# nannau/DoWnGAN

Hardware: AMD Instinct MI355X
Metric: train-step samples/sec (G+D+GP) (higher is better)
Workload: dtype bf16

## Files before the change

downgan_amd/csrc/conv_s2dgrad.hip:

```cpp
#include "gg_common.h"

namespace {

constexpr int NT = 512;
constexpr int RING_PIX = 17;
constexpr int RING_PITCH = 288;
constexpr int MASK_OFF = RING_PIX * RING_PITCH;
constexpr int RING_ROW = MASK_OFF + 2 * 32 * 16;
constexpr int RING_CHUNKS = RING_PIX * 16;

struct S2DArgs {
  const char* dy; const char* w; char* dx; const char* mask_bits;
  float slope;
  int Ho, Wo;
  int nstrips, nitems, trips;
};

__device__ __forceinline__ __amdgpu_buffer_rsrc_t uniform_rsrc(const char* p) {
  const unsigned long long b = (unsigned long long)p;
  const unsigned long long u = ((unsigned long long)(unsigned)__builtin_amdgcn_readfirstlane((int)(unsigned)(b >> 32)) << 32) |
                               (unsigned)__builtin_amdgcn_readfirstlane((int)(unsigned)b);
  return __builtin_amdgcn_make_buffer_rsrc((void*)u, 0, (int)DG_OOB_OFF, 0x00020000);
}

// ... 131 lines not shown
          store_pixel<MASK>(acc[0], acc[1], mb[0], a.slope, rY, st_lane + row0 * 256u);
        }
        {
          f32x4_t acc[2] = {f32x4_t{0.f, 0.f, 0.f, 0.f}, f32x4_t{0.f, 0.f, 0.f, 0.f}};
#pragma unroll
          for (int cb = 0; cb < 2; ++cb) {
            const uint4 b01[2] = {frag(sA, 1, cb, 0), frag(sA, 1, cb, 1)};
            tap(cb, 1, b01, acc); tap(cb, 2, b00[cb], acc);
          }
          store_pixel<MASK>(acc[0], acc[1], mb[1], a.slope, rY, st_lane + (row0 + 1) * 256u);
        }
        {
          f32x4_t acc[2] = {f32x4_t{0.f, 0.f, 0.f, 0.f}, f32x4_t{0.f, 0.f, 0.f, 0.f}};
#pragma unroll
          for (int cb = 0; cb < 2; ++cb) {
            const uint4 b10[2] = {frag(sB, 0, cb, 0), frag(sB, 0, cb, 1)};
            tap(cb, 3, b10, acc); tap(cb, 4, b00[cb], acc);
          }
          store_pixel<MASK>(acc[0], acc[1], mb[2], a.slope, rY, st_lane + (row0 + W) * 256u);
        }
      }
      if (filler) *reinterpret_cast<uint4*>(fill_dst + sC) = __builtin_bit_cast(uint4, staged);
      if (mwave) *reinterpret_cast<uint4*>(mfill_dst + sC) = __builtin_bit_cast(uint4, mstaged);
      __syncthreads();
      const int s = sA; sA = sB; sB = sC; sC = s;
    };
    for (int r = 0; r < a.Ho; r += 2) {
      step(r, st0, st1, ms0, ms1);
      if (r + 1 < a.Ho) step(r + 1, st1, st0, ms1, ms0);
    }
  }
}

std::atomic<int> g_s2_stream{1};
std::atomic<int> g_cus{0};

}

template <bool MASK>
__global__ __launch_bounds__(NT, 1) void s2dgrad_stream_kernel(const S2DArgs a) {
  __shared__ __attribute__((aligned(16))) char ring[3 * RING_ROW];
  if (__builtin_amdgcn_readfirstlane(threadIdx.x >> 6) < 4) s2d_run<MASK, true>(a, ring);
  else s2d_run<MASK, false>(a, ring);
}

bool s2dgrad_stream_eligible(const dg_conv_geom* g, const dg_epilogue* ep) {
  if (!g || g->dtype != DG_BF16 || g->stride != 2 || g->pixel_shuffle) return false;
  if (g->N <= 0 || g->H <= 0 || g->W <= 0 || ((g->H | g->W) & 1)) return false;
  if (g->Cin != 128 || g->Cout != 128 || g->ldx != 128 || g->ldy != 128) return false;
  if (!gg_halo_row_step_ok(g->W / 2, g->ldy, g->dtype, 1)) return false;
  if ((long long)g->H * g->W * 256 >= (1ll << 31)) return false;
  if (ep && (ep->bias || ep->has_act || ep->r1 || ep->r2 || ep->mask || ep->accumulate || ep->out_bits || ep->mask_c0 || ep->mask_last ||
             ep->out_q || ep->out_qs || ep->out_u || ep->out_ue || ep->skip_y || ep->out_amax))
    return false;
  return true;
}

int s2dgrad_stream_mode() { return g_s2_stream.load(std::memory_order_relaxed); }

extern "C" int dg_set_s2_dgrad_stream(int on) { return g_s2_stream.exchange(on < 0 ? 0 : on, std::memory_order_relaxed); }

int s2dgrad_stream_launch(const dg_conv_geom* g, const dg_epilogue* ep, const void* dy, const void* w, void* dx, hipStream_t st) {
  if (!dy || !w || !dx) return DG_ERR_BAD_ARG;
  int cus = g_cus.load(std::memory_order_relaxed);
  if (cus <= 0) {
    int dev = 0;
    if (hipGetDevice(&dev) != hipSuccess || hipDeviceGetAttribute(&cus, hipDeviceAttributeMultiprocessorCount, dev) != hipSuccess || cus <= 0)
      return DG_ERR_LAUNCH;
    g_cus.store(cus, std::memory_order_relaxed);
  }
  S2DArgs a{};
  a.dy = (const char*)dy; a.w = (const char*)w; a.dx = (char*)dx;
  a.mask_bits = ep ? (const char*)ep->mask_bits : nullptr;
  a.slope = ep ? ep->mask_slope : 1.f;
  a.Ho = g->H / 2; a.Wo = g->W / 2;
  a.nstrips = (a.Wo + 15) / 16;
  const long long items = (long long)g->N * a.nstrips;
  if (items >= (1ll << 31)) return DG_ERR_BAD_SHAPE;
  a.nitems = (int)items;
  const int mode = s2dgrad_stream_mode();
  int grid = mode > 1 && mode < cus ? mode : cus;
  if (grid > a.nitems) grid = a.nitems;
  a.trips = (a.nitems + grid - 1) / grid;
  g_last_kinds |= 64;
  if (a.mask_bits) hipLaunchKernelGGL(s2dgrad_stream_kernel<true>, dim3(grid), dim3(NT), 0, st, a);
  else hipLaunchKernelGGL(s2dgrad_stream_kernel<false>, dim3(grid), dim3(NT), 0, st, a);
  return dg_check_launch();
}
```

downgan_amd/_lib.py:

```python
from __future__ import annotations

import ctypes as C
import os

_HERE = os.path.dirname(os.path.abspath(__file__))
LIB_PATH = os.environ.get("DG_LIB_OVERRIDE") or os.path.join(_HERE, "csrc", "libdowngan_hip.so")

DG_F32, DG_BF16 = 0, 1
STATUS = {0: "DG_OK", -1: "DG_ERR_BAD_SHAPE", -2: "DG_ERR_BAD_DTYPE", -3: "DG_ERR_BAD_ARG", -4: "DG_ERR_LAUNCH"}


class Epilogue(C.Structure):
    _fields_ = [("bias", C.c_void_p), ("has_act", C.c_int), ("act_slope", C.c_float),
                ("r1", C.c_void_p), ("ldr1", C.c_int64), ("s1", C.c_float),
                ("r2", C.c_void_p), ("ldr2", C.c_int64), ("s2", C.c_float),
                ("mask", C.c_void_p), ("ldmask", C.c_int64), ("mask_slope", C.c_float),
                ("accumulate", C.c_int), ("mask_bits", C.c_void_p), ("out_bits", C.c_void_p),
                ("mask_c0", C.c_int), ("mask_last", C.c_int), ("out_q", C.c_void_p), ("out_qs", C.c_void_p), ("ldqs", C.c_int64),
                ("out_u", C.c_void_p), ("out_ue", C.c_void_p), ("skip_y", C.c_int), ("out_amax", C.c_void_p)]


class ConvGeom(C.Structure):
    _fields_ = [("dtype", C.c_int), ("N", C.c_int), ("H", C.c_int), ("W", C.c_int),
                ("Cin", C.c_int), ("Cout", C.c_int), ("stride", C.c_int), ("cin_real", C.c_int), ("pixel_shuffle", C.c_int),
# ... 103 lines not shown


class DistmapSpec(C.Structure):
    _fields_ = [("speed_u", C.c_int), ("speed_v", C.c_int), ("nthr", C.c_int), ("nring", C.c_int), ("cutoff", C.c_int),
                ("scale", C.c_float * EOF_MAX_C), ("offset", C.c_float * EOF_MAX_C),
                ("thr", (C.c_float * DIST_MAX_THR) * HIST_MAX_OUT)]


class TemporalSpec(C.Structure):
    _fields_ = [("speed_u", C.c_int), ("speed_v", C.c_int), ("nthr", C.c_int), ("ndur", C.c_int), ("nlag", C.c_int),
                ("nbins", C.c_int), ("below", C.c_int * TEMPORAL_MAX_THR), ("lag", C.c_int * TEMPORAL_MAX_LAGS),
                ("scale", C.c_float * EOF_MAX_C), ("offset", C.c_float * EOF_MAX_C),
                ("thr", (C.c_float * TEMPORAL_MAX_THR) * HIST_MAX_OUT), ("lo", (C.c_float * TEMPORAL_MAX_LAGS) * HIST_MAX_OUT),
                ("inv_w", (C.c_float * TEMPORAL_MAX_LAGS) * HIST_MAX_OUT)]


MINMAX_PARTS = 256
_vp, _i, _i64, _f = C.c_void_p, C.c_int, C.c_int64, C.c_float
_PROTOS = {
    "dg_conv3x3_fwd": [C.POINTER(ConvGeom), C.POINTER(Epilogue), _vp, _vp, _vp, _vp],
    "dg_conv3x3_dgrad": [C.POINTER(ConvGeom), C.POINTER(Epilogue), _vp, _vp, _vp, _vp],
    "dg_conv3x3_wgrad": [C.POINTER(ConvGeom), _vp, _vp, _vp, _vp, _vp],
    "dg_conv3x3_wgrad_dense": [_vp, _i, _vp, _vp, _vp, _vp, _vp],
    "dg_conv3x3_wgrad_f8": [C.POINTER(ConvGeom), _vp, _vp, _vp, _vp, _vp, _vp],
    "dg_exp_from_amax": [_vp, _i, _i, _vp, _vp],
    "dg_conv3x3_wgrad_dense_f8": [C.POINTER(ConvGeom), _i, _vp, _vp, _vp, _vp, _vp, _vp],
    "dg_gather_gemm": [C.POINTER(GGDesc), C.POINTER(Epilogue), _vp, _vp, _vp, _vp],
    "dg_conv3x3_plan": [C.POINTER(ConvGeom), _i, C.POINTER(GGDesc)],
    "dg_last_conv_kernels": [],
    "dg_last_wgrad_kernel": [],
    "dg_conv3x3_dgrad_launches": [C.POINTER(ConvGeom)],
    "dg_conv3x3_dgrad_stream_eligible": [C.POINTER(ConvGeom), C.POINTER(Epilogue)],
    "dg_set_s2_dgrad_stream": [C.c_int],
    "dg_colsum": [_i, _vp, _i64, _i64, _i64, _i64, _i, _vp, _vp],
    "dg_colsum_multi": [_i, _vp, _i64, _i64, _i, _i, _vp, _vp],
    "dg_repack_conv_weights": [_i, _i, _vp, _vp, _i, _i, _vp],
    "dg_repack_dense_dgrad": [_i, _vp, _i, _i, _vp, _vp],
    "dg_wgrad_unswap": [_vp, _vp, _i, _i, _vp],
    "dg_linear_fwd": [_i, _vp, _i64, _vp, _i64, _vp, _i, _i, _i, _i64, _vp],
    "dg_linear_dx": [_i, _i, _vp, _i, _vp, _i64, _vp, _i64, _vp, _i64, _f, _i, _i, _i64, _vp],
    "dg_linear_dw": [_i, _vp, _i, _vp, _i64, _vp, _i64, _i, _i, _i64, _vp],
    "dg_linear_dw_wide": [_i, _vp, _i, _vp, _i64, _vp, _i64, _i, _i, _i64, _i, _vp],
    "dg_bias_act": [_i, _vp, _i, _vp, _vp, _i, _i, _i, _i, _f, _vp, _i, _f, _vp],
    "dg_mask_mul": [_i, _vp, _i64, _vp, _i64, _i64, _i, _f, _vp],
    "dg_axpby": [_i, _vp, _i64, _vp, _i64, _f, _vp, _i64, _f, _i64, _i, _vp],
    "dg_gp_interp": [_i, _vp, _vp, _vp, _vp, _i, _i64, _vp],
    "dg_gp_interp_c2": [_i, _vp, _vp, _i64, _vp, _vp, _vp, _vp, _i, _i64, _vp],
    "dg_scale_rows_c2": [_i, _vp, _i64, _vp, _vp, _i, _i64, _vp],
    "dg_sumsq_rows": [_i, _vp, _i, _i64, _vp, _vp],
    "dg_gp_finish": [_vp, _i, _i, _f, _f, _vp, _vp, _vp],
    "dg_scale_rows": [_i, _vp, _vp, _vp, _i, _i64, _vp],
    "dg_l1": [_i, _vp, _i64, _vp, _i64, _i64, _i, _vp, _vp, _i64, _f, _vp, _i64, _vp],
    "dg_sqdiff": [_i, _vp, _i64, _vp, _i64, _i64, _i, _vp, _vp],
    "dg_sum_strided": [_vp, _i, _i, _f, _vp, _vp],
    "dg_fill_col": [_vp, _i, _i, _i, _f, _vp],
    "dg_adam": [_vp, _vp, _vp, _vp, _vp, _i64, _f, _f, _f, _f, _i, _f, _vp],
    "dg_nchw_to_nhwc": [_i, _vp, _vp, _i, _i, _i, _i, _i, _vp],
    "dg_nhwc_to_nchw": [_i, _vp, _i64, _vp, _i, _i, _i, _i, _vp],
    "dg_cast": [_i, _vp, _vp, _i64, _vp],
    "dg_minmax_partial": [_i, _vp, _i64, _i64, _i, _vp, _vp],
    "dg_minmax_finish": [_vp, _i, _vp, _vp],
    "dg_normalise_planar": [_i, _vp, _i, _i, _i, _i64, _i, _vp, _vp, _vp],
    "dg_ssim_level": [_vp, _vp, _i, _i, _i, C.POINTER(SsimParams), _vp, _vp],
    "dg_avgpool2": [_vp, _vp, _i, _i, _i, _vp],
    "dg_msssim_finish": [_vp, _i, _i, C.POINTER(MsssimCombine), _vp, _vp],
    "dg_div_vort_sums": [_i, _vp, _i64, _vp, _i64, _i, _i, _i, _vp, _vp],
# ... 127 lines not shown
```

downgan_amd/csrc/linear.hip:

```cpp
#include "dg_internal.h"
#include <stdlib.h>

template <typename T> struct MmaL;
template <> struct MmaL<bf16_t> {
  static __device__ __forceinline__ void run(const uint4& a, const uint4& b, f32x4_t& c) {
    c = __builtin_amdgcn_mfma_f32_16x16x32_bf16(__builtin_bit_cast(bf16x8_t, a), __builtin_bit_cast(bf16x8_t, b), c, 0, 0, 0);
  }
};
template <> struct MmaL<float> {
  static __device__ __forceinline__ void run(const uint4& a, const uint4& b, f32x4_t& c) {
    c = __builtin_amdgcn_mfma_f32_16x16x4f32(__uint_as_float(a.x), __uint_as_float(b.x), c, 0, 0, 0);
    c = __builtin_amdgcn_mfma_f32_16x16x4f32(__uint_as_float(a.y), __uint_as_float(b.y), c, 0, 0, 0);
    c = __builtin_amdgcn_mfma_f32_16x16x4f32(__uint_as_float(a.z), __uint_as_float(b.z), c, 0, 0, 0);
    c = __builtin_amdgcn_mfma_f32_16x16x4f32(__uint_as_float(a.w), __uint_as_float(b.w), c, 0, 0, 0);
  }
};

typedef __attribute__((ext_vector_type(2))) float dg_f32x2_t;
template <typename T> struct LdX4;
typedef __attribute__((ext_vector_type(2))) unsigned int dg_u32x2_t;
template <> struct LdX4<float> {
  typedef dg_u32x4_t raw;
  static __device__ __forceinline__ raw load(const float* row, unsigned voff) {
    return __builtin_amdgcn_raw_buffer_load_b128(__builtin_amdgcn_make_buffer_rsrc((void*)row, 0, -1, 0x00020000), voff, 0, 0);
// ... 224 lines not shown
        acc[4 * q + e][0] = __builtin_elementwise_fma(d2, wa, acc[4 * q + e][0]);
        acc[4 * q + e][1] = __builtin_elementwise_fma(d2, wb, acc[4 * q + e][1]);
      }
  };
  auto wrow = [&](int o) { return LdX4<T>::load(w + (long long)(o < O ? o : O - 1) * ldw, voff); };
  constexpr int PD = 6;
  typename LdX4<T>::raw wq[PD];
#pragma unroll
  for (int u = 0; u < PD; ++u) wq[u] = wrow(u);
  read_row(d[0], 0);
  for (int o = 0; o < O; o += PD) {
#pragma unroll
    for (int u = 0; u < PD; ++u) {
      read_row(d[(u + 1) & 1], o + u + 1 < O ? o + u + 1 : O);
      landed(d[u & 1]);
      row_fma(wq[u], d[u & 1]);
      wq[u] = wrow(o + u + PD);
    }
  }
#pragma unroll
  for (int b = 0; b < BG; ++b) {
    if (b0 + b >= B) break;
    float v[4] = {acc[b][0][0], acc[b][0][1], acc[b][1][0], acc[b][1][1]};
    if (mask) {
      float mv[4];
      ld4(mask + (long long)(b0 + b) * ldmask + k, mv);
#pragma unroll
      for (int e = 0; e < 4; ++e) v[e] *= leaky_grad(mv[e], slope);
    }
    st4(dx + (long long)(b0 + b) * lddx + k, v);
  }
}

extern "C" int dg_linear_dx(int dtype, int out_dtype, const float* dy, int ldo, const void* w, int64_t ldw, void* dx,
                            int64_t lddx, const void* mask, int64_t ldmask, float mask_slope, int B, int O, int64_t K,
                            void* stream) {
  if (!dy || !w || !dx) return DG_ERR_BAD_ARG;
  if (B <= 0 || O <= 0 || O > 128 || K <= 0 || K % 8 || ldw % 8 || lddx % 8) return DG_ERR_BAD_SHAPE;
  if (mask && ldmask % 8) return DG_ERR_BAD_SHAPE;
  hipStream_t st = reinterpret_cast<hipStream_t>(stream);
  if (K >= 4096 && (long long)K * 4 < (1ll << 32) && B >= 16) {
    dim3 gridw((unsigned)((K / 4 + 255) / 256), (unsigned)((B + 31) / 32));
    if (dtype == DG_F32 && out_dtype == DG_F32) {
      hipLaunchKernelGGL((lin_dx_wide_kernel<float, float>), gridw, dim3(256), 0, st, dy, ldo, (const float*)w, (long long)ldw, (float*)dx,
                         (long long)lddx, (const float*)mask, (long long)ldmask, mask_slope, B, O, (long long)K);
      return dg_check_launch();
    }
    if (dtype == DG_BF16 && out_dtype == DG_BF16) {
      hipLaunchKernelGGL((lin_dx_wide_kernel<bf16_t, bf16_t>), gridw, dim3(256), 0, st, dy, ldo, (const bf16_t*)w, (long long)ldw, (bf16_t*)dx,
                         (long long)lddx, (const bf16_t*)mask, (long long)ldmask, mask_slope, B, O, (long long)K);
      return dg_check_launch();
    }
  }
  constexpr int BG = 16;
  const int epc = dtype == DG_F32 ? 4 : 8;
  dim3 grid((unsigned)((K / epc + 255) / 256), (unsigned)((B + BG - 1) / BG));
  if (dtype == DG_F32 && out_dtype == DG_F32)
    hipLaunchKernelGGL((lin_dx_kernel<float, float, BG>), grid, dim3(256), 0, st, dy, ldo, (const float*)w, ldw,
                       (float*)dx, lddx, (const float*)mask, ldmask, mask_slope, B, O, K);
  else if (dtype == DG_BF16 && out_dtype == DG_BF16)
    hipLaunchKernelGGL((lin_dx_kernel<bf16_t, bf16_t, BG>), grid, dim3(256), 0, st, dy, ldo, (const bf16_t*)w, ldw,
                       (bf16_t*)dx, lddx, (const bf16_t*)mask, ldmask, mask_slope, B, O, K);
  else if (dtype == DG_BF16 && out_dtype == DG_F32)
    hipLaunchKernelGGL((lin_dx_kernel<bf16_t, float, BG>), grid, dim3(256), 0, st, dy, ldo, (const bf16_t*)w, ldw,
                       (float*)dx, lddx, (const bf16_t*)mask, ldmask, mask_slope, B, O, K);
  else
    return DG_ERR_BAD_DTYPE;
  return dg_check_launch();
}

template <typename T, int OT>
__global__ __launch_bounds__(256) void lin_dw_kernel(const float* __restrict__ dy, int ldo, const T* __restrict__ x,
                                                     long long ldx, float* dw, long long lddw, int B, int O,
// ... 84 lines not shown
      for (int j = 0; j < OW; ++j) {
        const float dv = dp[j];
        const dg_f32x2_t d2 = {dv, dv};
        acc[j][0] = __builtin_elementwise_fma(d2, xa, acc[j][0]);
        acc[j][1] = __builtin_elementwise_fma(d2, xb, acc[j][1]);
      }
    };
    const int Bm = B / (2 * UB) * (2 * UB);
    fetch(0, 0);
    for (int b0 = 0; b0 < Bm; b0 += 2 * UB) {
      fetch(1, b0 + UB);
#pragma unroll
      for (int u = 0; u < UB; ++u) row_fma(xr[0][u], b0 + u);
      fetch(0, b0 + 2 * UB);
#pragma unroll
      for (int u = 0; u < UB; ++u) row_fma(xr[1][u], b0 + UB + u);
    }
    for (int b = Bm; b < B; ++b) row_fma(LdX4<T>::load(x + (long long)b * ldx, voff), b);
#pragma unroll
    for (int j = 0; j < OW; ++j) {
      const int o = wave * OW + j;
      if (o >= O) break;
      float4* p = reinterpret_cast<float4*>(dw + (long long)o * lddw + k);
      float4 t = make_float4(acc[j][0][0], acc[j][0][1], acc[j][1][0], acc[j][1][1]);
      if (ACC) {
        const float4 old = *p;
        t.x += old.x; t.y += old.y; t.z += old.z; t.w += old.w;
      }
      *p = t;
    }
  }
}

extern "C" int dg_linear_dw_wide(int dtype, const float* dy, int ldo, const void* x, int64_t ldx, float* dw, int64_t lddw,
                                 int B, int O, int64_t K, int accumulate, void* stream) {
  if (!dy || !x || !dw) return DG_ERR_BAD_ARG;
  if (B <= 0 || B > 128 || O <= 0 || O > 112 || ldo < 112 || K <= 0 || K >= (1ll << 30) || K % 4 || ldx % 4 || lddw % 4 || ldx < K || lddw < K)
    return DG_ERR_BAD_SHAPE;
  if (dtype != DG_F32 && dtype != DG_BF16) return DG_ERR_BAD_DTYPE;
  hipStream_t st = reinterpret_cast<hipStream_t>(stream);
  const long long chunks = (K + 255) / 256;
  const int cpw = chunks >= 8 * 2048 ? 8 : chunks >= 2048 ? 2 : 1;
  const unsigned grid = (unsigned)((chunks + cpw - 1) / cpw);
  constexpr int NWV = 8;
#define DG_LDW(T, ACC)                                                                                                  \
  hipLaunchKernelGGL((lin_dw_wide_kernel<T, ACC, NWV>), dim3(grid), dim3(64 * NWV), 0, st, dy, ldo, (const T*)x, \
                     (long long)ldx, dw, (long long)lddw, B, O, (long long)K, cpw)
  if (dtype == DG_F32) { if (accumulate) DG_LDW(float, true); else DG_LDW(float, false); }
  else { if (accumulate) DG_LDW(bf16_t, true); else DG_LDW(bf16_t, false); }
#undef DG_LDW
  return dg_check_launch();
}
```

include/downgan_hip.h:

```cpp
#ifndef DOWNGAN_HIP_H
#define DOWNGAN_HIP_H

#include <stddef.h>
#include <stdint.h>

#ifdef __cplusplus
extern "C" {
#endif

#define DG_F32 0
#define DG_BF16 1

typedef enum dg_status {
  DG_OK = 0,
  DG_ERR_BAD_SHAPE = -1,
  DG_ERR_BAD_DTYPE = -2,
  DG_ERR_BAD_ARG = -3,
  DG_ERR_LAUNCH = -4
} dg_status;

typedef struct dg_epilogue {
  const float* bias;
  int has_act;
  float act_slope;
// ... 47 lines not shown
                     const void* w_dgrad, void* dx, void* stream);

int dg_conv3x3_wgrad(const dg_conv_geom* g, const void* x, const void* dy, float* dw, float* db,
                     void* stream);

int dg_conv3x3_wgrad_dense(const dg_conv_geom* g, int nconv, const void* x, const void* dy,
                           float* const* dw, float* const* db, void* stream);

int dg_conv3x3_wgrad_f8(const dg_conv_geom* g, const void* xq, const void* ex, const void* dyq, const void* ey, float* dw,
                        void* stream);

int dg_conv3x3_wgrad_dense_f8(const dg_conv_geom* g, int nconv, const void* xq, const void* ex, const void* dyq, const void* ey,
                              float* const* dw, void* stream);

int dg_colsum(int dtype, const void* dy, int64_t rows_outer, int64_t ld_outer, int64_t rows_inner,
              int64_t ld, int C, float* db, void* stream);

int dg_colsum_multi(int dtype, const void* dy, int64_t rows, int64_t ld, int C, int nseg, float* const* db, void* stream);

int dg_gather_gemm(const dg_gg_desc* d, const dg_epilogue* ep, const void* x, const void* w, void* y,
                   void* stream);

int dg_last_conv_kernels(void);

int dg_last_wgrad_kernel(void);

int dg_conv3x3_plan(const dg_conv_geom* g, int kind, dg_gg_desc* out);

int dg_conv3x3_dgrad_launches(const dg_conv_geom* g);

int dg_conv3x3_dgrad_stream_eligible(const dg_conv_geom* g, const dg_epilogue* ep);

int dg_set_s2_dgrad_stream(int on);

int dg_repack_conv_weights(int dtype, int kind, const float* master, void* dst, int CoutP, int CinP,
                           void* stream);
int dg_repack_dense_dgrad(int dtype, const float* const* masters, int nconv, int F, void* dst, void* stream);
int dg_wgrad_unswap(const float* tmp, float* dw, int CoutP, int CinP, void* stream);


int dg_linear_fwd(int dtype, const void* x, int64_t ldx, const void* w, int64_t ldw, float* y,
                  int ldy, int B, int O, int64_t K, void* stream);
int dg_linear_dx(int dtype, int out_dtype, const float* dy, int ldo, const void* w, int64_t ldw,
                 void* dx, int64_t lddx, const void* mask, int64_t ldmask, float mask_slope, int B,
                 int O, int64_t K, void* stream);
int dg_linear_dw(int dtype, const float* dy, int ldo, const void* x, int64_t ldx, float* dw,
                 int64_t lddw, int B, int O, int64_t K, void* stream);
int dg_linear_dw_wide(int dtype, const float* dy, int ldo, const void* x, int64_t ldx, float* dw,
                      int64_t lddw, int B, int O, int64_t K, int accumulate, void* stream);


int dg_bias_act(int out_dtype, const float* in, int ldi, const float* bias, void* out, int ldo,
                int rows, int C, int has_act, float slope, const void* mask, int ldmask,
                float mask_slope, void* stream);
int dg_mask_mul(int dtype, void* u, int64_t ldu, const void* y, int64_t ldy, int64_t rows, int C,
                float slope, void* stream);
int dg_axpby(int dtype, void* out, int64_t ldo, const void* x, int64_t ldx, float a, const void* y,
             int64_t ldy, float b, int64_t rows, int C, void* stream);
int dg_gp_interp(int dtype, const void* real, const void* fake, const float* alpha, void* xhat,
                 int B, int64_t per_img, void* stream);
int dg_gp_interp_c2(int dtype, const void* real, const void* fake, int64_t ld, const float* alpha,
                    void* xhat_c, void* real_c, void* fake_c, int B, int64_t pix_per_img, void* stream);
int dg_scale_rows_c2(int dtype, const void* g, int64_t ld, const float* coef, void* out_c, int B,
                     int64_t pix_per_img, void* stream);
int dg_sumsq_rows(int dtype, const void* g, int B, int64_t per_img, float* ss, void* stream);
int dg_gp_finish(const float* ss, int B, int B_global, float gp_lambda, float weight, float* coef,
// ... 283 lines not shown
```

Baseline: 73.77.

## Add streaming stride-2 dgrad kernel for 256-channel convolutions

Extends the streaming stride-2 transposed-conv data-gradient kernel to Cin=Cout=256, which previously fell back to another path. Each block handles one 64-output-channel slice of a strip and keeps that slice's weights in registers, reloading them only when the slice changes. Row ring buffering in LDS overlaps the next row's load with the MMA work. Work is assigned per XCD so blocks on the same die share strips. The cost is heavy register use for the weight fragments, plus four passes over the input strip, one per channel slice.

After: 73.95 (median of 3 runs). About the same (+0.2%).

```diff
diff --git a/downgan_amd/csrc/conv_s2dgrad.hip b/downgan_amd/csrc/conv_s2dgrad.hip
--- a/downgan_amd/csrc/conv_s2dgrad.hip
+++ b/downgan_amd/csrc/conv_s2dgrad.hip
@@ -187,6 +187,197 @@
   }
 }
 
+constexpr int R2_PITCH = 544;
+constexpr int R2_MASK_OFF = RING_PIX * R2_PITCH;
+constexpr int R2_ROW = R2_MASK_OFF + 2 * 32 * 8;
+
+struct S2D256Args {
+  const char* dy; const char* w; char* dx; const char* mask_bits;
+  float slope;
+  int Ho, Wo;
+  int nstrips, npairs, trips;
+  int per_xcd;
+};
+
+template <bool MASK>
+__device__ __forceinline__ void store_pixel4(const f32x4_t& f, unsigned nib, float slope, __amdgpu_buffer_rsrc_t rY, unsigned off) {
+  float v[4] = {f[0], f[1], f[2], f[3]};
+  if (MASK) {
+#pragma unroll
+    for (int e = 0; e < 4; ++e) v[e] *= ((nib >> e) & 1u) ? 1.f : slope;
+  }
+  EpiIO<bf16_t>::store(v, rY, off);
+}
+
+template <bool MASK, bool C11>
+__device__ __forceinline__ void s2d256_run(const S2D256Args& a, char* ring) {
+  constexpr int NTAP = C11 ? 4 : 5;
+  const int tid = threadIdx.x, lane = tid & 63, q = (tid >> 6) & 3;
+  const int l15 = lane & 15, g = lane >> 4;
+
+  uint4 wr[NTAP * 8];
+  int wslice = -1;
+
+  const int W = 2 * a.Wo;
+  const char* const fb0 = ring + l15 * R2_PITCH + g * 16;
+  const int fill_pix = tid >> 5;
+  char* const fill_dst = ring + fill_pix * R2_PITCH + (tid & 31) * 16;
+  const bool xfiller = C11 && tid < 32;
+  char* const xfill_dst = ring + 16 * R2_PITCH + (tid & 31) * 16;
+
+  for (int trip = 0; trip < a.trips; ++trip) {
+    int pair, s;
+    if (a.per_xcd > 0) {
+      const int j = (int)blockIdx.x >> 3;
+      s = j & 3;
+      pair = (trip * a.per_xcd + (j >> 2)) * 8 + ((int)blockIdx.x & 7);
+    } else {
+      const int item = (int)blockIdx.x + trip * (int)gridDim.x;
+      s = item & 3;
+      pair = item >> 2;
+    }
+    if (pair >= a.npairs) break;
+    if (s != wslice) {
+      wslice = s;
+      constexpr int TW11[4] = {0, 2, 6, 8}, TWX[5] = {4, 3, 5, 1, 7};
+      const int n = 64 * s + 16 * q + l15;
+#pragma unroll
+      for (int cb = 0; cb < 4; ++cb)
+#pragma unroll
+        for (int t = 0; t < NTAP; ++t)
+#pragma unroll
+          for (int kk = 0; kk < 2; ++kk) {
+            const int tw = C11 ? TW11[t] : TWX[t];
+            wr[(cb * NTAP + t) * 2 + kk] =
+                *reinterpret_cast<const uint4*>(a.w + ((long long)n * 2304 + tw * 256 + 64 * cb + 32 * kk + 8 * g) * 2);
+          }
+    }
+    const int img = pair / a.nstrips, x0 = (pair - img * a.nstrips) * 16;
+    const __amdgpu_buffer_rsrc_t rX = uniform_rsrc(a.dy + ((long long)img * a.Ho * a.Wo + x0) * 512);
+    const __amdgpu_buffer_rsrc_t rY = uniform_rsrc(a.dx + ((long long)img * 2 * a.Ho * W + 2 * x0) * 512);
+    const __amdgpu_buffer_rsrc_t rM = uniform_rsrc(MASK ? a.mask_bits + ((long long)img * 2 * a.Ho * W + 2 * x0) * 32 : a.dx);
+    const unsigned fill_off = x0 + fill_pix < a.Wo ? (unsigned)tid * 16u : DG_OOB_OFF;
+    const unsigned xfill_off = (xfiller && x0 + 16 < a.Wo) ? (unsigned)(16 * 512 + tid * 16) : DG_OOB_OFF;
+    const unsigned pix_ok = x0 + l15 < a.Wo ? 0u : DG_OOB_OFF;
+    const unsigned st_lane = pix_ok | (unsigned)(2 * l15 * 512 + 128 * s + 32 * q + 8 * g);
+    auto fetch_row = [&](unsigned off, int rr) {
+      return __builtin_amdgcn_raw_buffer_load_b128(rX, rr < a.Ho ? off + (unsigned)rr * (unsigned)a.Wo * 512u : DG_OOB_OFF, 0, 0);
+    };
+    const bool mwave = MASK && !C11 && __builtin_amdgcn_readfirstlane(tid >> 6) == 5;
+    const int ml = tid & 63;
+    const unsigned mfill_off = 2 * x0 + (ml & 31) < W ? (unsigned)(((ml >> 5) * W + (ml & 31)) * 32 + 8 * s) : DG_OOB_OFF;
+    char* const mfill_dst = ring + R2_MASK_OFF + ml * 8;
+    auto fetch_mask = [&](int k) {
+      return __builtin_amdgcn_raw_buffer_load_b64(rM, k < a.Ho ? mfill_off + (unsigned)(2 * k) * (unsigned)W * 32u : DG_OOB_OFF, 0, 0);
+    };
+    const char* const mrd = ring + R2_MASK_OFF + 2 * l15 * 8 + 2 * q + (g >> 1);
+    const unsigned nsh = 4u * (unsigned)(g & 1);
+    {
+      const u32x4_t r0 = fetch_row(fill_off, 0), r1 = fetch_row(fill_off, 1);
+      *reinterpret_cast<uint4*>(fill_dst) = __builtin_bit_cast(uint4, r0);
+      *reinterpret_cast<uint4*>(fill_dst + R2_ROW) = __builtin_bit_cast(uint4, r1);
+      if constexpr (C11) {
+        const u32x4_t x0r = fetch_row(xfill_off, 0), x1r = fetch_row(xfill_off, 1);
+        if (xfiller) {
+          *reinterpret_cast<uint4*>(xfill_dst) = __builtin_bit_cast(uint4, x0r);
+          *reinterpret_cast<uint4*>(xfill_dst + R2_ROW) = __builtin_bit_cast(uint4, x1r);
+        }
+      }
+      if (mwave) *reinterpret_cast<uint2*>(mfill_dst + R2_ROW) = __builtin_bit_cast(uint2, fetch_mask(0));
+    }
+    u32x4_t st0 = fetch_row(fill_off, 2), st1;
+    u32x4_t xs0 = {0u, 0u, 0u, 0u}, xs1 = {0u, 0u, 0u, 0u};
+    if (xfiller) xs0 = fetch_row(xfill_off, 2);
+    u32x2_t ms0 = {0u, 0u}, ms1 = {0u, 0u};
+    if (mwave) ms0 = fetch_mask(1);
+    __syncthreads();
+    int sA = 0, sB = R2_ROW, sC = 2 * R2_ROW;
+    auto step = [&](int r, const u32x4_t& staged, u32x4_t& nxt, const u32x4_t& xstaged, u32x4_t& xnxt, const u32x2_t& mstaged,
+                    u32x2_t& mnxt) __attribute__((always_inline)) {
+      nxt = fetch_row(fill_off, r + 3);
+      if (xfiller) xnxt = fetch_row(xfill_off, r + 3);
+      if (mwave) mnxt = fetch_mask(r + 2);
+      unsigned mb[3] = {0u, 0u, 0u};
+      if (MASK) {
+        if (C11) {
+          mb[0] = *reinterpret_cast<const unsigned char*>(mrd + sB + 256 + 8);
+        } else {
+          mb[0] = *reinterpret_cast<const unsigned char*>(mrd + sB);
+          mb[1] = *reinterpret_cast<const unsigned char*>(mrd + sB + 8);
+          mb[2] = *reinterpret_cast<const unsigned char*>(mrd + sB + 256);
+        }
+      }
+      const unsigned row0 = (unsigned)(2 * r) * (unsigned)W;
+      __builtin_amdgcn_sched_barrier(0);
+      auto frag = [&](int slot, int sx, int cb, int kk) {
+        return *reinterpret_cast<const uint4*>(fb0 + slot + sx * R2_PITCH + cb * 128 + kk * 64);
+      };
+      if constexpr (C11) {
+        f32x4_t acc = {0.f, 0.f, 0.f, 0.f};
+        uint4 b[2][8];
+        auto read = [&](int cb) {
+#pragma unroll
+          for (int t = 0; t < 4; ++t)
+#pragma unroll
+            for (int kk = 0; kk < 2; ++kk) b[cb & 1][t * 2 + kk] = frag(t < 2 ? sB : sA, (t & 1) ? 0 : 1, cb, kk);
+        };
+        read(0);
+#pragma unroll
+        for (int cb = 0; cb < 4; ++cb) {
+          if (cb < 3) read(cb + 1);
+          __builtin_amdgcn_sched_barrier(0);
+#pragma unroll
+          for (int i = 0; i < 8; ++i) Mma<bf16_t>::run(wr[cb * 8 + i], b[cb & 1][i], acc);
+          __builtin_amdgcn_sched_barrier(0);
+        }
+        store_pixel4<MASK>(acc, mb[0] >> nsh, a.slope, rY, st_lane + (row0 + W + 1) * 512u);
+      } else {
+        f32x4_t a00 = {0.f, 0.f, 0.f, 0.f}, a01 = {0.f, 0.f, 0.f, 0.f}, a10 = {0.f, 0.f, 0.f, 0.f};
+        uint4 b[2][6];
+        auto read = [&](int cb) {
+#pragma unroll
+          for (int kk = 0; kk < 2; ++kk) {
+            b[cb & 1][kk] = frag(sA, 0, cb, kk);
+            b[cb & 1][2 + kk] = frag(sA, 1, cb, kk);
+            b[cb & 1][4 + kk] = frag(sB, 0, cb, kk);
+          }
+        };
+        read(0);
+#pragma unroll
+        for (int cb = 0; cb < 4; ++cb) {
+          if (cb < 3) read(cb + 1);
+          __builtin_amdgcn_sched_barrier(0);
+          const uint4* const bc = b[cb & 1];
+#pragma unroll
+          for (int kk = 0; kk < 2; ++kk) {
+            Mma<bf16_t>::run(wr[cb * 10 + 0 + kk], bc[kk], a00);
+            Mma<bf16_t>::run(wr[cb * 10 + 2 + kk], bc[2 + kk], a01);
+            Mma<bf16_t>::run(wr[cb * 10 + 6 + kk], bc[4 + kk], a10);
+          }
+#pragma unroll
+          for (int kk = 0; kk < 2; ++kk) {
+            Mma<bf16_t>::run(wr[cb * 10 + 4 + kk], bc[kk], a01);
+            Mma<bf16_t>::run(wr[cb * 10 + 8 + kk], bc[kk], a10);
+          }
+          __builtin_amdgcn_sched_barrier(0);
+        }
+        store_pixel4<MASK>(a00, mb[0] >> nsh, a.slope, rY, st_lane + row0 * 512u);
+        store_pixel4<MASK>(a01, mb[1] >> nsh, a.slope, rY, st_lane + (row0 + 1) * 512u);
+        store_pixel4<MASK>(a10, mb[2] >> nsh, a.slope, rY, st_lane + (row0 + W) * 512u);
+      }
+      *reinterpret_cast<uint4*>(fill_dst + sC) = __builtin_bit_cast(uint4, staged);
+      if (xfiller) *reinterpret_cast<uint4*>(xfill_dst + sC) = __builtin_bit_cast(uint4, xstaged);
+      if (mwave) *reinterpret_cast<uint2*>(mfill_dst + sC) = __builtin_bit_cast(uint2, mstaged);
+      __syncthreads();
+      const int sw = sA; sA = sB; sB = sC; sC = sw;
+    };
+    for (int r = 0; r < a.Ho; r += 2) {
+      step(r, st0, st1, xs0, xs1, ms0, ms1);
+      if (r + 1 < a.Ho) step(r + 1, st1, st0, xs1, xs0, ms1, ms0);
+    }
+  }
+}
+
 std::atomic<int> g_s2_stream{1};
 std::atomic<int> g_cus{0};
 
@@ -199,12 +390,19 @@
   else s2d_run<MASK, false>(a, ring);
 }
 
+template <bool MASK>
+__global__ __launch_bounds__(NT, 1) void s2dgrad_stream256_kernel(const S2D256Args a) {
+  __shared__ __attribute__((aligned(16))) char ring[3 * R2_ROW];
+  if (__builtin_amdgcn_readfirstlane(threadIdx.x >> 6) < 4) s2d256_run<MASK, true>(a, ring);
+  else s2d256_run<MASK, false>(a, ring);
+}
+
 bool s2dgrad_stream_eligible(const dg_conv_geom* g, const dg_epilogue* ep) {
   if (!g || g->dtype != DG_BF16 || g->stride != 2 || g->pixel_shuffle) return false;
   if (g->N <= 0 || g->H <= 0 || g->W <= 0 || ((g->H | g->W) & 1)) return false;
-  if (g->Cin != 128 || g->Cout != 128 || g->ldx != 128 || g->ldy != 128) return false;
+  if ((g->Cin != 128 && g->Cin != 256) || g->Cout != g->Cin || g->ldx != g->Cin || g->ldy != g->Cin) return false;
   if (!gg_halo_row_step_ok(g->W / 2, g->ldy, g->dtype, 1)) return false;
-  if ((long long)g->H * g->W * 256 >= (1ll << 31)) return false;
+  if ((long long)g->H * g->W * g->Cin * 2 >= (1ll << 31)) return false;
   if (ep && (ep->bias || ep->has_act || ep->r1 || ep->r2 || ep->mask || ep->accumulate || ep->out_bits || ep->mask_c0 || ep->mask_last ||
              ep->out_q || ep->out_qs || ep->out_u || ep->out_ue || ep->skip_y || ep->out_amax))
     return false;
@@ -223,6 +421,27 @@
     if (hipGetDevice(&dev) != hipSuccess || hipDeviceGetAttribute(&cus, hipDeviceAttributeMultiprocessorCount, dev) != hipSuccess || cus <= 0)
       return DG_ERR_LAUNCH;
     g_cus.store(cus, std::memory_order_relaxed);
+  }
+  const int mode = s2dgrad_stream_mode();
+  if (g->Cin == 256) {
+    S2D256Args a{};
+    a.dy = (const char*)dy; a.w = (const char*)w; a.dx = (char*)dx;
+    a.mask_bits = ep ? (const char*)ep->mask_bits : nullptr;
+    a.slope = ep ? ep->mask_slope : 1.f;
+    a.Ho = g->H / 2; a.Wo = g->W / 2;
+    a.nstrips = (a.Wo + 15) / 16;
+    const long long pairs = (long long)g->N * a.nstrips;
+    if (pairs >= (1ll << 28)) return DG_ERR_BAD_SHAPE;
+    a.npairs = (int)pairs;
+    const int items = 4 * a.npairs;
+    int grid = mode > 1 && mode < cus ? mode : cus;
+    if (grid > items) grid = items;
+    a.per_xcd = grid % 32 == 0 ? grid / 32 : 0;
+    a.trips = a.per_xcd ? (a.npairs + grid / 4 - 1) / (grid / 4) : (items + grid - 1) / grid;
+    g_last_kinds |= 64;
+    if (a.mask_bits) hipLaunchKernelGGL(s2dgrad_stream256_kernel<true>, dim3(grid), dim3(NT), 0, st, a);
+    else hipLaunchKernelGGL(s2dgrad_stream256_kernel<false>, dim3(grid), dim3(NT), 0, st, a);
+    return dg_check_launch();
   }
   S2DArgs a{};
   a.dy = (const char*)dy; a.w = (const char*)w; a.dx = (char*)dx;
@@ -233,7 +452,6 @@
   const long long items = (long long)g->N * a.nstrips;
   if (items >= (1ll << 31)) return DG_ERR_BAD_SHAPE;
   a.nitems = (int)items;
-  const int mode = s2dgrad_stream_mode();
   int grid = mode > 1 && mode < cus ? mode : cus;
   if (grid > a.nitems) grid = a.nitems;
   a.trips = (a.nitems + grid - 1) / grid;
```

## Add MFMA paths for wide linear dx and dw using three-way bf16 splitting

Applied to the files above, without the earlier changes.

Adds MFMA-based kernels for the linear-layer input gradient and the wide weight gradient in bf16. The fp32 dy operand is split into three bf16 terms so the product keeps near-fp32 accuracy, and weight/activation tiles are staged in LDS with a prefetch of the next tile and read with transposed LDS loads. This replaces the scalar FMA row kernels for large K, trading three MFMAs per product and extra LDS traffic for matrix-core throughput. A runtime switch, on by default, allows either path to be disabled.

Result: no change. 73.84 before, 73.98 after, median of 6 (+0.2%).

```diff
diff --git a/downgan_amd/_lib.py b/downgan_amd/_lib.py
--- a/downgan_amd/_lib.py
+++ b/downgan_amd/_lib.py
@@ -159,6 +159,7 @@
     "dg_conv3x3_dgrad_launches": [C.POINTER(ConvGeom)],
     "dg_conv3x3_dgrad_stream_eligible": [C.POINTER(ConvGeom), C.POINTER(Epilogue)],
     "dg_set_s2_dgrad_stream": [C.c_int],
+    "dg_set_linear_mfma": [C.c_int],
     "dg_colsum": [_i, _vp, _i64, _i64, _i64, _i64, _i, _vp, _vp],
     "dg_colsum_multi": [_i, _vp, _i64, _i64, _i, _i, _vp, _vp],
     "dg_repack_conv_weights": [_i, _i, _vp, _vp, _i, _i, _vp],
diff --git a/downgan_amd/csrc/linear.hip b/downgan_amd/csrc/linear.hip
--- a/downgan_amd/csrc/linear.hip
+++ b/downgan_amd/csrc/linear.hip
@@ -280,6 +280,156 @@
   }
 }
 
+constexpr int MX_KT = 256, MX_PITCH = 2 * MX_KT + 16, MX_ROWS = 128;
+constexpr int MX_LDS = MX_ROWS * MX_PITCH;
+#define MX_OOB 0x80000000u
+__device__ __forceinline__ __amdgpu_buffer_rsrc_t mx_rsrc(const void* p) {
+  return __builtin_amdgcn_make_buffer_rsrc((void*)p, 0, (int)MX_OOB, 0x00020000);
+}
+__device__ __forceinline__ bf16x8_t mx_read_tr16(const unsigned char* lo_p, const unsigned char* hi_p) {
+  typedef __attribute__((address_space(3))) s16x4_t* lds_s16x4_ptr;
+  typedef __attribute__((ext_vector_type(8))) short s16x8_t;
+  const s16x4_t lo = __builtin_amdgcn_ds_read_tr16_b64_v4i16((lds_s16x4_ptr)(lo_p));
+  const s16x4_t hi = __builtin_amdgcn_ds_read_tr16_b64_v4i16((lds_s16x4_ptr)(hi_p));
+  const s16x8_t v = {lo[0], lo[1], lo[2], lo[3], hi[0], hi[1], hi[2], hi[3]};
+  return __builtin_bit_cast(bf16x8_t, v);
+}
+__device__ __forceinline__ void mx_split3(const float (&v)[8], bf16x8_t (&t)[3]) {
+  unsigned h[3][8];
+#pragma unroll
+  for (int j = 0; j < 8; ++j) {
+    float r = v[j];
+#pragma unroll
+    for (int s = 0; s < 3; ++s) {
+      h[s][j] = __float_as_uint(r) & 0xffff0000u;
+      r -= __uint_as_float(h[s][j]);
+    }
+  }
+#pragma unroll
+  for (int s = 0; s < 3; ++s) {
+    const dg_u32x4_t p = {(h[s][0] >> 16) | h[s][1], (h[s][2] >> 16) | h[s][3], (h[s][4] >> 16) | h[s][5], (h[s][6] >> 16) | h[s][7]};
+    t[s] = __builtin_bit_cast(bf16x8_t, p);
+  }
+}
+__device__ __forceinline__ void mx_st16(bf16_t* p, const float* v, bool lo, bool hi) {
+  if (lo) *reinterpret_cast<uint4*>(p) = make_uint4(pack_bf16x2(v[0], v[1]), pack_bf16x2(v[2], v[3]), pack_bf16x2(v[4], v[5]), pack_bf16x2(v[6], v[7]));
+  if (hi) *reinterpret_cast<uint4*>(p + 8) = make_uint4(pack_bf16x2(v[8], v[9]), pack_bf16x2(v[10], v[11]), pack_bf16x2(v[12], v[13]), pack_bf16x2(v[14], v[15]));
+}
+__device__ __forceinline__ void mx_st16(float* p, const float* v, bool lo, bool hi) {
+#pragma unroll
+  for (int q = 0; q < 4; ++q)
+    if (q < 2 ? lo : hi) *reinterpret_cast<float4*>(p + 4 * q) = make_float4(v[4 * q], v[4 * q + 1], v[4 * q + 2], v[4 * q + 3]);
+}
+
+template <typename TO>
+__global__ __launch_bounds__(256, 2) void lin_dx_mfma_kernel(const float* __restrict__ dy, int ldo, const bf16_t* __restrict__ w,
+                                                             long long ldw, TO* dx, long long lddx, const bf16_t* mask,
+                                                             long long ldmask, float slope, int B, int O, long long K, int ntiles) {
+  extern __shared__ __attribute__((aligned(16))) unsigned char mx_smem[];
+  const int tid = threadIdx.x, lane = tid & 63, wave = tid >> 6;
+  const int l15 = lane & 15, g = lane >> 4;
+  const int b0 = blockIdx.y * 32;
+  bf16x8_t dq[4][2][3];
+#pragma unroll
+  for (int ob = 0; ob < 4; ++ob)
+#pragma unroll
+    for (int f = 0; f < 2; ++f) {
+      const int b = b0 + 16 * f + l15;
+      float v[8];
+#pragma unroll
+      for (int j = 0; j < 8; ++j) {
+        const int o = 32 * ob + 8 * g + j;
+        v[j] = (b < B && o < O) ? dy[(long long)b * ldo + o] : 0.f;
+      }
+      mx_split3(v, dq[ob][f]);
+    }
+  for (int i = tid; i < 16 * MX_PITCH / 16; i += 256) *reinterpret_cast<uint4*>(mx_smem + 112 * MX_PITCH + 16 * i) = make_uint4(0u, 0u, 0u, 0u);
+  const int r0 = tid >> 5, c = tid & 31;
+  const unsigned rowstep = (unsigned)(8 * ldw * 2);
+  const unsigned voff0 = (unsigned)(r0 * ldw * 2) + 16u * c;
+  uint4 stg[14];
+  auto fetch = [&](int tile) {
+    const long long k0 = (long long)tile * MX_KT;
+    const __amdgpu_buffer_rsrc_t rs = mx_rsrc(w + k0);
+    const bool kin = k0 + 8 * c < K;
+#pragma unroll
+    for (int i = 0; i < 14; ++i) {
+      const bool ok = kin && r0 + 8 * i < O;
+      const dg_u32x4_t t = __builtin_amdgcn_raw_buffer_load_b128(rs, ok ? voff0 + (unsigned)i * rowstep : MX_OOB, 0, 0);
+      stg[i] = make_uint4(t[0], t[1], t[2], t[3]);
+    }
+  };
+  const unsigned char* const abase = mx_smem + (8 * g + (l15 >> 2)) * MX_PITCH + 2 * (64 * wave + 16 * (l15 & 3));
+  int tile = blockIdx.x;
+  if (tile < ntiles) fetch(tile);
+  for (; tile < ntiles; tile += gridDim.x) {
+    __syncthreads();
+#pragma unroll
+    for (int i = 0; i < 14; ++i) *reinterpret_cast<uint4*>(mx_smem + (r0 + 8 * i) * MX_PITCH + 16 * c) = stg[i];
+    __syncthreads();
+    const long long kk = (long long)tile * MX_KT + 64 * wave + 16 * g;
+    const bool klo = kk < K, khi = kk + 8 < K;
+    uint4 mk[2][2];
+    if (mask) {
+#pragma unroll
+      for (int f = 0; f < 2; ++f) {
+        const int b = b0 + 16 * f + l15;
+        const bf16_t* mp = mask + (long long)b * ldmask + kk;
+        mk[f][0] = (b < B && klo) ? *reinterpret_cast<const uint4*>(mp) : make_uint4(0u, 0u, 0u, 0u);
+        mk[f][1] = (b < B && khi) ? *reinterpret_cast<const uint4*>(mp + 8) : make_uint4(0u, 0u, 0u, 0u);
+      }
+    }
+    if (tile + (int)gridDim.x < ntiles) fetch(tile + (int)gridDim.x);
+    f32x4_t acc[4][2];
+#pragma unroll
+    for (int t = 0; t < 4; ++t) acc[t][0] = acc[t][1] = f32x4_t{0.f, 0.f, 0.f, 0.f};
+#pragma unroll
+    for (int t = 0; t < 4; ++t)
+#pragma unroll
+      for (int ob = 0; ob < 4; ++ob) {
+        const unsigned char* pa = abase + 32 * ob * MX_PITCH + 8 * t;
+        const bf16x8_t a = mx_read_tr16(pa, pa + 4 * MX_PITCH);
+#pragma unroll
+        for (int f = 0; f < 2; ++f)
+#pragma unroll
+          for (int s = 2; s >= 0; --s) acc[t][f] = __builtin_amdgcn_mfma_f32_16x16x32_bf16(a, dq[ob][f][s], acc[t][f], 0, 0, 0);
+      }
+#pragma unroll
+    for (int f = 0; f < 2; ++f) {
+      const int b = b0 + 16 * f + l15;
+      if (b >= B) continue;
+      float v[16];
+#pragma unroll
+      for (int t = 0; t < 4; ++t)
+#pragma unroll
+        for (int e = 0; e < 4; ++e) v[4 * t + e] = acc[t][f][e];
+      if (mask) {
+        const unsigned m[8] = {mk[f][0].x, mk[f][0].y, mk[f][0].z, mk[f][0].w, mk[f][1].x, mk[f][1].y, mk[f][1].z, mk[f][1].w};
+#pragma unroll
+        for (int q = 0; q < 8; ++q) {
+          v[2 * q] *= leaky_grad(__uint_as_float(m[q] << 16), slope);
+          v[2 * q + 1] *= leaky_grad(__uint_as_float(m[q] & 0xffff0000u), slope);
+        }
+      }
+      mx_st16(dx + (long long)b * lddx + kk, v, klo, khi);
+    }
+  }
+}
+
+static std::atomic<int> g_lin_mfma{3};
+extern "C" int dg_set_linear_mfma(int on) { return g_lin_mfma.exchange(on < 0 ? 0 : on, std::memory_order_relaxed); }
+
+template <typename TO>
+static int lin_dx_mfma_launch(const float* dy, int ldo, const bf16_t* w, long long ldw, TO* dx, long long lddx, const bf16_t* mask,
+                              long long ldmask, float slope, int B, int O, long long K, hipStream_t st) {
+  DG_SET_MAX_LDS_ONCE((lin_dx_mfma_kernel<TO>), MX_LDS);
+  const long long ntiles = (K + MX_KT - 1) / MX_KT;
+  const unsigned gx = (unsigned)(ntiles < 512 ? ntiles : 512);
+  hipLaunchKernelGGL((lin_dx_mfma_kernel<TO>), dim3(gx, (unsigned)((B + 31) / 32)), dim3(256), MX_LDS, st, dy, ldo, w, ldw, dx, lddx,
+                     mask, ldmask, slope, B, O, K, (int)ntiles);
+  return dg_check_launch();
+}
+
 extern "C" int dg_linear_dx(int dtype, int out_dtype, const float* dy, int ldo, const void* w, int64_t ldw, void* dx,
                             int64_t lddx, const void* mask, int64_t ldmask, float mask_slope, int B, int O, int64_t K,
                             void* stream) {
@@ -287,6 +437,16 @@
   if (B <= 0 || O <= 0 || O > 128 || K <= 0 || K % 8 || ldw % 8 || lddx % 8) return DG_ERR_BAD_SHAPE;
   if (mask && ldmask % 8) return DG_ERR_BAD_SHAPE;
   hipStream_t st = reinterpret_cast<hipStream_t>(stream);
+  if (K >= 4096 && (long long)K * 4 < (1ll << 32)) {
+    if (dtype == DG_BF16 && (out_dtype == DG_BF16 || out_dtype == DG_F32) && O <= 112 && ldw > 0 &&
+        (long long)(O + 7) * ldw * 2 + 2 * MX_KT < (long long)MX_OOB && (g_lin_mfma.load(std::memory_order_relaxed) & 1)) {
+      if (out_dtype == DG_BF16)
+        return lin_dx_mfma_launch<bf16_t>(dy, ldo, (const bf16_t*)w, (long long)ldw, (bf16_t*)dx, (long long)lddx, (const bf16_t*)mask,
+                                          (long long)ldmask, mask_slope, B, O, (long long)K, st);
+      return lin_dx_mfma_launch<float>(dy, ldo, (const bf16_t*)w, (long long)ldw, (float*)dx, (long long)lddx, (const bf16_t*)mask,
+                                       (long long)ldmask, mask_slope, B, O, (long long)K, st);
+    }
+  }
   if (K >= 4096 && (long long)K * 4 < (1ll << 32) && B >= 16) {
     dim3 gridw((unsigned)((K / 4 + 255) / 256), (unsigned)((B + 31) / 32));
     if (dtype == DG_F32 && out_dtype == DG_F32) {
@@ -437,6 +597,95 @@
   }
 }
 
+constexpr int DWM_KT = 128, DWM_PITCH = 2 * DWM_KT + 16, DWM_NT = 448, DWM_CH = 5;
+constexpr int DWM_LDS = (DWM_CH * DWM_NT / 16) * DWM_PITCH;
+template <bool ACC>
+__global__ __launch_bounds__(DWM_NT, 4) void lin_dw_mfma_kernel(const float* __restrict__ dy, int ldo, const bf16_t* __restrict__ x,
+                                                                long long ldx, float* dw, long long lddw, int B, int O,
+                                                                long long K, int ntiles) {
+  extern __shared__ __attribute__((aligned(16))) unsigned char mx_smem[];
+  const int tid = threadIdx.x, lane = tid & 63, wave = tid >> 6;
+  const int l15 = lane & 15, g = lane >> 4;
+  const int nbb = (B + 31) >> 5;
+  const int o = 16 * wave + l15;
+  bf16x8_t dq[4][3];
+#pragma unroll
+  for (int bb = 0; bb < 4; ++bb) {
+    float v[8];
+#pragma unroll
+    for (int j = 0; j < 8; ++j) {
+      const int b = 32 * bb + 8 * g + j;
+      v[j] = (b < B && o < O) ? dy[(long long)b * ldo + o] : 0.f;
+    }
+    mx_split3(v, dq[bb]);
+  }
+  unsigned voff[DWM_CH];
+#pragma unroll
+  for (int i = 0; i < DWM_CH; ++i) {
+    const int id = tid + DWM_NT * i, row = id >> 4;
+    voff[i] = row < B ? (unsigned)(row * ldx * 2) + 16u * (id & 15) : MX_OOB;
+  }
+  uint4 stg[DWM_CH];
+  auto fetch = [&](int tile) {
+    const long long k0 = (long long)tile * DWM_KT;
+    const __amdgpu_buffer_rsrc_t rs = mx_rsrc(x + k0);
+    const bool kin = k0 + 8 * (tid & 15) < K;
+#pragma unroll
+    for (int i = 0; i < DWM_CH; ++i) {
+      const dg_u32x4_t t = __builtin_amdgcn_raw_buffer_load_b128(rs, kin ? voff[i] : MX_OOB, 0, 0);
+      stg[i] = make_uint4(t[0], t[1], t[2], t[3]);
+    }
+  };
+  const unsigned char* const abase = mx_smem + (8 * g + (l15 >> 2)) * DWM_PITCH + 2 * 16 * (l15 & 3);
+  int tile = blockIdx.x;
+  if (tile < ntiles) fetch(tile);
+  for (; tile < ntiles; tile += gridDim.x) {
+    __syncthreads();
+#pragma unroll
+    for (int i = 0; i < DWM_CH; ++i) {
+      const int id = tid + DWM_NT * i;
+      *reinterpret_cast<uint4*>(mx_smem + (id >> 4) * DWM_PITCH + 16 * (id & 15)) = stg[i];
+    }
+    __syncthreads();
+    if (tile + (int)gridDim.x < ntiles) fetch(tile + (int)gridDim.x);
+    f32x4_t acc[2][4];
+#pragma unroll
+    for (int h = 0; h < 2; ++h)
+#pragma unroll
+      for (int t = 0; t < 4; ++t) acc[h][t] = f32x4_t{0.f, 0.f, 0.f, 0.f};
+#pragma unroll
+    for (int bb = 0; bb < 4; ++bb) {
+      if (bb >= nbb) break;
+#pragma unroll
+      for (int h = 0; h < 2; ++h)
+#pragma unroll
+        for (int t = 0; t < 4; ++t) {
+          const unsigned char* pa = abase + 32 * bb * DWM_PITCH + 2 * 64 * h + 8 * t;
+          const bf16x8_t a = mx_read_tr16(pa, pa + 4 * DWM_PITCH);
+#pragma unroll
+          for (int s = 2; s >= 0; --s) acc[h][t] = __builtin_amdgcn_mfma_f32_16x16x32_bf16(a, dq[bb][s], acc[h][t], 0, 0, 0);
+        }
+    }
+    if (o < O) {
+#pragma unroll
+      for (int h = 0; h < 2; ++h) {
+        const long long kk = (long long)tile * DWM_KT + 64 * h + 16 * g;
+        float4* p = reinterpret_cast<float4*>(dw + (long long)o * lddw + kk);
+#pragma unroll
+        for (int t = 0; t < 4; ++t) {
+          if (kk + 4 * t >= K) break;
+          float4 r = make_float4(acc[h][t][0], acc[h][t][1], acc[h][t][2], acc[h][t][3]);
+          if (ACC) {
+            const float4 old = p[t];
+            r.x += old.x; r.y += old.y; r.z += old.z; r.w += old.w;
+          }
+          p[t] = r;
+        }
+      }
+    }
+  }
+}
+
 extern "C" int dg_linear_dw_wide(int dtype, const float* dy, int ldo, const void* x, int64_t ldx, float* dw, int64_t lddw,
                                  int B, int O, int64_t K, int accumulate, void* stream) {
   if (!dy || !x || !dw) return DG_ERR_BAD_ARG;
@@ -444,6 +693,21 @@
     return DG_ERR_BAD_SHAPE;
   if (dtype != DG_F32 && dtype != DG_BF16) return DG_ERR_BAD_DTYPE;
   hipStream_t st = reinterpret_cast<hipStream_t>(stream);
+  if (dtype == DG_BF16 && K % 8 == 0 && ldx % 8 == 0 && (long long)B * ldx * 2 + 2 * DWM_KT < (long long)MX_OOB &&
+      (g_lin_mfma.load(std::memory_order_relaxed) & 2)) {
+    const long long ntiles = (K + DWM_KT - 1) / DWM_KT;
+    const unsigned gx = (unsigned)(ntiles < 512 ? ntiles : 512);
+    if (accumulate) {
+      DG_SET_MAX_LDS_ONCE((lin_dw_mfma_kernel<true>), DWM_LDS);
+      hipLaunchKernelGGL((lin_dw_mfma_kernel<true>), dim3(gx), dim3(DWM_NT), DWM_LDS, st, dy, ldo, (const bf16_t*)x, (long long)ldx, dw,
+                         (long long)lddw, B, O, (long long)K, (int)ntiles);
+    } else {
+      DG_SET_MAX_LDS_ONCE((lin_dw_mfma_kernel<false>), DWM_LDS);
+      hipLaunchKernelGGL((lin_dw_mfma_kernel<false>), dim3(gx), dim3(DWM_NT), DWM_LDS, st, dy, ldo, (const bf16_t*)x, (long long)ldx, dw,
+                         (long long)lddw, B, O, (long long)K, (int)ntiles);
+    }
+    return dg_check_launch();
+  }
   const long long chunks = (K + 255) / 256;
   const int cpw = chunks >= 8 * 2048 ? 8 : chunks >= 2048 ? 2 : 1;
   const unsigned grid = (unsigned)((chunks + cpw - 1) / cpw);
diff --git a/include/downgan_hip.h b/include/downgan_hip.h
--- a/include/downgan_hip.h
+++ b/include/downgan_hip.h
@@ -103,6 +103,8 @@
 int dg_conv3x3_dgrad_stream_eligible(const dg_conv_geom* g, const dg_epilogue* ep);
 
 int dg_set_s2_dgrad_stream(int on);
+
+int dg_set_linear_mfma(int on);
 
 int dg_repack_conv_weights(int dtype, int kind, const float* master, void* dst, int CoutP, int CinP,
                            void* stream);
```
